# SohirMaskey/raincast-gnn

Hardware: AMD Instinct MI355X
Metric: training graphs/s (24h_mixed GNN, full train step) (higher is better)
Workload: dtype f32 (split-bf16x3 GEMM products, fp32 accumulate); 1 GPU; cfg2: 24h_mixed, 32 graphs x 500 stations, k=10, 4 GINE layers, D=128; global_batch=32, graphs_per_gpu=32, nodes_per_gpu=16000, edges_per_gpu=176000, parallelism=dp1, hip_graph=True, station_order=locality, allreduce_in_graph=False, allreduce_overlap=False, head_fold=True

## Files before the change

### raincast-gnn_amd/csrc/gine_chain.hip

```cpp
#include "gine_common.hpp"
#include "gine_slab.hpp"
#include "gine_wgrad.hpp"
#include "gine_chainfold.hpp"
#include "gine_chainrow.hpp"

#include <algorithm>

namespace gine {
namespace {

typedef float floatx16 __attribute__((ext_vector_type(16)));

constexpr int kRowTile = 32;

#ifdef GINE_CHAIN_PROFILE
__device__ long long g_chain_prof[1024][16];
#define CHAIN_MARK(i)                                                          \
  do {                                                                         \
    if (threadIdx.x == 0 && blockIdx.x < 1024)                                 \
      g_chain_prof[blockIdx.x][i] = (long long)__builtin_amdgcn_s_memtime();  \
  } while (0)
#define CHAIN_RT(i)                                                            \
  do {                                                                         \
    if (threadIdx.x == 0 && blockIdx.x < 1024)                                 \
// ... 74 lines not shown
    const int c = k < F ? k : (k < FP ? 0 : k - FP + F);
    const float v = WT[(size_t)c * D + col];
    bf[s] = (k >= F && k < FP) ? 0.f : v;
  }
}

struct TileRange {
  int first, end, step;
};
__device__ __forceinline__ TileRange tile_range(int num_tiles, int nb) {
  const int xcd = blockIdx.x % kNumXcd, pos = blockIdx.x / kNumXcd;
  const int here = nb / kNumXcd + (xcd < nb % kNumXcd ? 1 : 0);
  const int span = (num_tiles + kNumXcd - 1) / kNumXcd;
  const int b = xcd * span;
  return TileRange{b + pos, min(num_tiles, b + span), here};
}

template <int D, int FP, int KIND>
__global__ __launch_bounds__(2 * D) void k_chain(ChainArgs a, int64_t N, int num_tiles) {
  constexpr int NT = 2 * D;
  constexpr int D4 = D / 4;
  constexpr int LDA = D + 4;
  constexpr bool kDimRed = KIND == CH_F2;
  constexpr int K2 = kDimRed ? FP + D : D;
  constexpr int LDB = K2 + 4;
  constexpr int BOFF = kDimRed ? FP : 0;
  constexpr int ITEMS = kRowTile * D4 / NT;
  constexpr int RSTEP = NT / D4;
  constexpr int XITEMS = (kRowTile * FP + NT - 1) / NT;
  constexpr bool kF2D = KIND == CH_F2D, kB2D = KIND == CH_B2D;
  constexpr bool kMask = KIND == CH_B1 || kB2D;
  constexpr bool kX = kDimRed || kF2D;
  constexpr int LDC = FP + D + 4;
  __shared__ __attribute__((aligned(16))) float sA[kRowTile * LDA];
  __shared__ __attribute__((aligned(16))) float sB[kF2D ? 4 : kRowTile * LDB];
  __shared__ __attribute__((aligned(16))) float sC[kF2D ? kRowTile * LDC : 4];

  const int wave = threadIdx.x / kWave, lane = threadIdx.x % kWave;
  const int h = lane >> 5, c32 = lane & 31;
  const int col = wave * 32 + c32;
  const int q_me = threadIdx.x % D4, r_me = threadIdx.x / D4;
  CHAIN_RT(11);
  CHAIN_MARK(0);
  const int nb = gridDim.x;

  float bf1[D / 2], bf2[K2 / 2];
  const bool w16 =
      ((reinterpret_cast<uintptr_t>(a.w1) | reinterpret_cast<uintptr_t>(a.w2)) & 15) == 0;
  if constexpr (KIND == CH_F1) {
    if (w16) {
      frag_t4<D>(bf1, a.w1, D, col, h);
      frag_t4<D>(bf2, a.w2, D, col, h);
    } else {
      frag_t<D>(bf1, a.w1, D, col, h);
      frag_t<D>(bf2, a.w2, D, col, h);
    }
  } else if constexpr (kF2D) {
    if (w16) frag_t4<D>(bf1, a.w1, D, col, h);
    else frag_t<D>(bf1, a.w1, D, col, h);
  } else if constexpr (KIND == CH_F2) {
    frag_t<D>(bf1, a.w1, D, col, h);
  } else if constexpr (kMask) {
    frag_n<D>(bf1, a.w1, a.F + D, a.F, col, h);
  } else if constexpr (KIND == CH_B2) {
    frag_n<D>(bf1, a.w1, D, 0, col, h);
  }
// ... 51 lines not shown
    for (int i = 0; i < ITEMS; ++i) {
      const int r = r_me + i * RSTEP;
      const float4 v = (n0 + r < N) ? raw[i] : f4_zero();
      float* dst = &sA[r * LDA + 4 * q_me];
      *reinterpret_cast<float4*>(dst) = v;
    }
    if constexpr (kX) {
      float* sx = kF2D ? sC : sB;
      constexpr int LDX = kF2D ? LDC : LDB;
#pragma unroll
      for (int i = 0; i < XITEMS; ++i) {
        const int idx = threadIdx.x + i * NT;
        if (idx < kRowTile * FP) sx[(idx / FP) * LDX + idx % FP] = idx % FP < a.F ? xr[i] : 0.f;
      }
    }
    __syncthreads();
    if (kt < 2) CHAIN_MARK(2 + 4 * kt);
    if (tile + tr.step < tr.end) load_tile(tile + tr.step, raw, xr);

    floatx16 acc;
    acc = tile_mma<D>(sA, LDA, bf1, c32, h);
#pragma unroll
    for (int r = 0; r < 16; ++r) {
      const int rr = (r & 3) + 8 * (r >> 2) + 4 * h;
      const int64_t n = n0 + rr;
      float v = acc[r] + bias1;
      if constexpr (kB2D) v = ep[r] > 0.f ? acc[r] : 0.f;
      if constexpr (kF2D) {
        v = relu_nan(v);
        sC[rr * LDC + FP + col] = v;
      } else {
        sB[rr * LDB + BOFF + col] = v;
      }
      if (n < N) a.out1[n * D + col] = v;
    }
    if (kt < 2) CHAIN_MARK(3 + 4 * kt);
    __syncthreads();
    if (kt < 2) CHAIN_MARK(4 + 4 * kt);

    if constexpr (!kF2D) {
      acc = tile_mma<K2>(sB, LDB, bf2, c32, h);
#pragma unroll
      for (int r = 0; r < 16; ++r) {
        const int rr = (r & 3) + 8 * (r >> 2) + 4 * h;
        const int64_t n = n0 + rr;
        float v = acc[r] + bias2;
        if constexpr (KIND == CH_F1) v = relu_nan(v);
        if constexpr (KIND == CH_B1) v = ep[r] > 0.f ? v : 0.f;
        if (n < N) a.out2[n * D + col] = v;
      }
    } else {
      acc = tile_mma<FP + D>(sC, LDC, bf3, c32, h);
#pragma unroll
      for (int r = 0; r < 16; ++r) {
        const int64_t n = n0 + (r & 3) + 8 * (r >> 2) + 4 * h;
        if (n < N) a.out3[n * D + col] = acc[r] + bias3;
      }
    }
    if (kt < 2) CHAIN_MARK(5 + 4 * kt);
  }
  CHAIN_MARK(10);
  CHAIN_RT(12);
}

inline int chain_grid(int64_t N) {
  const int64_t tiles = ceil_div(N, kRowTile);
  return (int)std::max<int64_t>(1, std::min<int64_t>(tiles, kNumCu));
}

template <int D, int FP, int KIND>
int launch_chain(const ChainArgs& a, int64_t N, hipStream_t s) {
  const int tiles = (int)ceil_div(N, kRowTile);
  hipLaunchKernelGGL((k_chain<D, FP, KIND>), dim3(chain_grid(N)), dim3(2 * D), 0, s, a, N,
                     tiles);
  GINE_LAUNCH_STATUS();
  return GINE_OK;
}

template <int NZ>
struct ChainWgradSrc {
  static constexpr int kZ = NZ;
  const float* p[NZ];
  const float* q[NZ];
  const float* x;
  int D, F;
  struct Raw {
    float4 v;
  };
  struct Col {
    float keep[4];
  };
  template <int Z> __device__ int i_dim(int) const { return Z == 0 ? F + D : D; }
  template <int Z> __device__ Col p_col(int) const { return Col{{1.f, 1.f, 1.f, 1.f}}; }
  template <int Z> __device__ Col q_col(int q4) const {
    Col c{{1.f, 1.f, 1.f, 1.f}};
    if constexpr (Z == 0) {
#pragma unroll
      for (int j = 0; j < 4; ++j) c.keep[j] = 4 * q4 + j < F + D ? 1.f : 0.f;
    }
    return c;
  }
  template <int Z> __device__ Raw p_load(int64_t n, int q4) const {
    return Raw{reinterpret_cast<const float4*>(p[Z] + n * D)[q4]};
  }
  template <int Z> __device__ Raw q_load(int64_t n, int q4) const {
    if constexpr (Z == 0) {
      const int I = F + D;
      float v[4];
#pragma unroll
      for (int j = 0; j < 4; ++j) {
        const int c = min(4 * q4 + j, I - 1);
        const float* src = c < F ? x + n * F + c : q[0] + n * D + (c - F);
        v[j] = *src;
      }
// ... 395 lines not shown
```

### raincast-gnn_amd/csrc/gine_common.hpp

```cpp
#pragma once

#include <hip/hip_runtime.h>
#include <stdint.h>

#include "gine_hip.h"

#define GINE_RETURN_IF_HIP(expr)                                  \
  do {                                                            \
    hipError_t gine_e_ = (expr);                                  \
    if (gine_e_ != hipSuccess) return GINE_ERR_HIP_BASE + (int)gine_e_; \
  } while (0)


#define GINE_LAUNCH_STATUS() \
  do {                                                            \
    hipError_t gine_e_ = hipGetLastError();                       \
    if (gine_e_ != hipSuccess) return GINE_ERR_HIP_BASE + (int)gine_e_; \
  } while (0)

namespace gine {

constexpr int kWave = 64;
constexpr int kNumXcd = 8;
constexpr int kNumCu = 256;

inline hipStream_t as_stream(void* s) { return reinterpret_cast<hipStream_t>(s); }

__device__ __forceinline__ int xcd_remap(int bid, int nblocks) {
  const int q = nblocks / kNumXcd, r = nblocks % kNumXcd;
  const int xcd = bid % kNumXcd, pos = bid / kNumXcd;
  const int base = (xcd < r) ? xcd * (q + 1) : r * (q + 1) + (xcd - r) * q;
  return base + pos;
}

__device__ __forceinline__ float4 f4_zero() { return make_float4(0.f, 0.f, 0.f, 0.f); }

__device__ __forceinline__ float relu_nan(float v) { return __builtin_elementwise_maximum(v, 0.0f); }

__device__ __forceinline__ bool block_any(bool pred, int* word) {
  __syncthreads();
  if (threadIdx.x == 0) *word = 0;
  __syncthreads();
  if (pred) *word = 1;
  __syncthreads();
  const bool any = *word != 0;
  __syncthreads();
  return any;
}

template <bool FMA>
__device__ __forceinline__ float edge_lin(float a, float w, float b) {
  if constexpr (FMA) return __builtin_fmaf(a, w, b);
  return a * w + b;
}

__device__ __forceinline__ double shfl_xor_d(double v, int m) {
  return __shfl_xor(v, m, kWave);
}

__host__ __device__ inline int64_t ceil_div(int64_t a, int64_t b) { return (a + b - 1) / b; }

__device__ __forceinline__ void count_valid_parts(const float* __restrict__ y, int64_t n,
                                                  uint32_t* __restrict__ parts) {
  __shared__ uint32_t s_w[4];
  const int64_t chunk = (n + GINE_COUNT_PARTS - 1) / GINE_COUNT_PARTS;
  for (int p = blockIdx.x; p < GINE_COUNT_PARTS; p += gridDim.x) {
    const int64_t lo = (int64_t)p * chunk, hi = lo + chunk < n ? lo + chunk : n;
    uint32_t c = 0;
// ... 11 lines not shown
```

### raincast-gnn_amd/csrc/gine_deepset.hip

```cpp
#include "gine_common.hpp"
#include "gine_chainfold.hpp"
#include "gine_bf16x3.hpp"
#include "gine_chainrow.hpp"

#include <algorithm>
#include <type_traits>

namespace gine {
namespace {

typedef float floatx16 __attribute__((ext_vector_type(16)));

__host__ __device__ constexpr int tiles_per_group(int G, int M) { return (G * M + 15) / 16; }

#ifndef GINE_DS_BF16X3
#define GINE_DS_BF16X3 1
#endif
template <int KP>
struct DsImg {
  static constexpr int KX = (KP + 15) / 16 * 16;
  static constexpr int RS = KX + 8;
  static constexpr int PLANE = 32 * RS;
  static constexpr int FLOATS = 3 * PLANE / 2;
};
// ... 472 lines not shown
  float bf[H / 2];
  frag_n<H>(bf, a.w1, a.FX + H, a.FX, col, h);
  float ep[16];
#pragma unroll
  for (int r = 0; r < 16; ++r) {
    int64_t n = n0 + (r & 3) + 8 * (r >> 2) + 4 * h;
    n = n < N ? n : N - 1;
    ep[r] = a.u[n * H + col];
  }
#pragma unroll
  for (int i = 0; i < ITEMS; ++i) {
    const int r = r_me + i * RSTEP;
    *reinterpret_cast<float4*>(&sA[r * LDA + 4 * q_me]) = (n0 + r < N) ? raw[i] : f4_zero();
  }
  __syncthreads();
  floatx16 acc = tile_mma<H>(sA, LDA, bf, c32, h);
#pragma unroll
  for (int r = 0; r < 16; ++r) {
    const int rr = (r & 3) + 8 * (r >> 2) + 4 * h;
    const float v = ep[r] > 0.f ? acc[r] : 0.f;
    sB[rr * LDA + col] = v;
    if (n0 + rr < N) a.dt[(n0 + rr) * H + col] = v;
  }
  frag_n<H>(bf, a.w2, H, 0, col, h);
  __syncthreads();
  acc = tile_mma<H>(sB, LDA, bf, c32, h);
#pragma unroll
  for (int r = 0; r < 16; ++r) {
    const int rr = (r & 3) + 8 * (r >> 2) + 4 * h;
    s_dr[rr * H + col] = n0 + rr < N ? acc[r] + 0.f : 0.f;
  }
}

template <int H, int KP, int G, bool X3, bool CHAIN = false>
__device__ __forceinline__ bool ds_bwd_body(const float* __restrict__ ens,
                                            const uint16_t* __restrict__ mask,
                                            const float* __restrict__ dr,
                                            float* __restrict__ slab, int64_t N, int M, int F,
                                            int num_groups, float* s_lds,
                                            const DsChainArgs& ch = DsChainArgs{}) {
  static_assert(!CHAIN || G == 16, "a group is one chain tile at G = 16 only");
  constexpr int NT = 2 * H;
  constexpr int KI = ds_bwd_ki(KP);
  using I = DsBwdImg<KI>;
  constexpr int LD = X3 ? I::RS : KP + 4;
  constexpr int TILEF = X3 ? I::FLOATS : 32 * (KP + 4);
  constexpr int NIF = X3 ? KI / 32 : KP / 32;
  constexpr int TAIL = X3 ? 0 : KP - 32 * NIF;
  float* s_e0 = s_lds;
  float* s_e1 = s_lds + TILEF;
  float* s_dr = s_lds + 2 * TILEF;
  const int wave = threadIdx.x / kWave, lane = threadIdx.x % kWave;
  const int h = lane >> 5, c32 = lane & 31;
  const int col = wave * 32 + c32;
  if constexpr (X3) {
    uint16_t* i0 = reinterpret_cast<uint16_t*>(s_e0);
    uint16_t* i1 = reinterpret_cast<uint16_t*>(s_e1);
    const int w = (KI - F) * I::RS;
    for (int i = threadIdx.x; i < 3 * w; i += blockDim.x) {
      const int pl = i / w, e = F * I::RS + i % w;
      i0[pl * I::PLANE + e] = 0;
      i1[pl * I::PLANE + e] = 0;
    }
  } else {
    zero_pad<KP>(s_e0, F);
    zero_pad<KP>(s_e1, F);
// ... 76 lines not shown
        const float* erow = buf + (16 * h + q) * LD;
#pragma unroll
        for (int it = 0; it < NIF; ++it)
          gw[it] = __builtin_amdgcn_mfma_f32_32x32x2f32(dh[q], erow[32 * it + c32], gw[it], 0,
                                                        0, 0);
#pragma unroll
        for (int j = 0; j < TAIL; j += 4) {
          const float4 e4 = *reinterpret_cast<const float4*>(erow + 32 * NIF + j);
          tw[j] = __builtin_fmaf(dh[q], e4.x, tw[j]);
          tw[j + 1] = __builtin_fmaf(dh[q], e4.y, tw[j + 1]);
          tw[j + 2] = __builtin_fmaf(dh[q], e4.z, tw[j + 2]);
          tw[j + 3] = __builtin_fmaf(dh[q], e4.w, tw[j + 3]);
        }
      }
    }
    DS_MARK(3 + 0 * (int)gw[0][0]);
  };
  if constexpr (CHAIN) {
    float* sA = s_dr + 2 * G * H;
    walk_tiles<true, true>(gr, GM, tpg, st, ens, N * M, F, s_e0, s_e1, mask, tile, [&]() {
      ds_chain_tile<H>(ch, N, (int64_t)gr.first * 2 * G, sA, sA + 32 * (H + 4), s_dr, wave,
                       c32, h);
    });
  } else {
    walk_tiles<true, true>(gr, GM, tpg, st, ens, N * M, F, s_e0, s_e1, mask, tile);
  }
  if constexpr (X3) {
    bool bad = false;
#pragma unroll
    for (int it = 0; it < NIF; ++it) bad = bad || wave_any_nan(gw[it]);
    if (block_any(bad, reinterpret_cast<int*>(s_e0))) return false;
  }
  float* out = slab + (size_t)blockIdx.x * ((size_t)H * F + H);
#pragma unroll
  for (int it = 0; it < NIF; ++it) {
#pragma unroll
    for (int q = 0; q < 16; ++q) {
      const int o = wave * 32 + (q & 3) + 8 * (q >> 2) + 4 * h;
      if (32 * it + c32 < F) out[(size_t)o * F + 32 * it + c32] = gw[it][q];
    }
  }
#pragma unroll
  for (int j = 0; j < TAIL; ++j) {
    const float v = tw[j] + __shfl_xor(tw[j], 32, kWave);
    if (h == 0 && 32 * NIF + j < F) out[(size_t)col * F + 32 * NIF + j] = v;
  }
  gb += shfl_xor_d(gb, 32);
  if (h == 0) out[(size_t)H * F + col] = (float)gb;
  return true;
}

#ifndef GINE_DS_BWD_BF16X3
#define GINE_DS_BWD_BF16X3 0
#endif
template <int H, int KP, int G>
constexpr int ds_bwd_lds_floats() {
  constexpr int f32 = 2 * 32 * (KP + 4);
  constexpr int x3 = GINE_DS_BWD_BF16X3 ? 2 * DsBwdImg<ds_bwd_ki(KP)>::FLOATS : 0;
  return (f32 > x3 ? f32 : x3) + 2 * G * H;
}

template <int H, int KP, int G>
__global__ __launch_bounds__(2 * H) void k_deepset_bwd(const float* __restrict__ ens,
                                                       const uint16_t* __restrict__ mask,
                                                       const float* __restrict__ dr,
                                                       float* __restrict__ slab, int64_t N,
                                                       int M, int F, int num_groups) {
  __shared__ __attribute__((aligned(16))) float s_lds[ds_bwd_lds_floats<H, KP, G>()];
#if GINE_DS_BWD_BF16X3
  if (ds_bwd_body<H, KP, G, true>(ens, mask, dr, slab, N, M, F, num_groups, s_lds)) return;
  __syncthreads();
#endif
  ds_bwd_body<H, KP, G, false>(ens, mask, dr, slab, N, M, F, num_groups, s_lds);
}

template <int H, int KP>
__global__ __launch_bounds__(2 * H) void k_deepset_bwd_chain(const float* __restrict__ ens,
                                                             const uint16_t* __restrict__ mask,
                                                             DsChainArgs ch,
                                                             float* __restrict__ slab, int64_t N,
                                                             int M, int F, int num_groups) {
  __shared__ __attribute__((aligned(16)))
  float s_lds[ds_bwd_lds_floats<H, KP, 16>() + ds_chain_lds_floats<H>()];
#if GINE_DS_BWD_BF16X3
  if (ds_bwd_body<H, KP, 16, true, true>(ens, mask, nullptr, slab, N, M, F, num_groups, s_lds,
                                         ch))
    return;
  __syncthreads();
#endif
  ds_bwd_body<H, KP, 16, false, true>(ens, mask, nullptr, slab, N, M, F, num_groups, s_lds, ch);
}

// ... 322 lines not shown
```

### raincast-gnn_amd/csrc/gine_mpmlp.hip

```cpp
#include "gine_mpmlp.hpp"

namespace gine {
namespace {

template <bool FMA>
__global__ __launch_bounds__(kThreads, 1) void k_mp_fwd_mlp1(FusedArgs A) {
  __shared__ __attribute__((aligned(16))) FusedLds L;
  const TileSeq ts = tile_seq(A.num_tiles, blockIdx.x, gridDim.x);
  const int nt = ts.count();
  const int wave = __builtin_amdgcn_readfirstlane(threadIdx.x / kWave);
  if (wave < kMatThreads / kWave) matrix_role(A, L, ts, nt);
  else gather_role<FMA>(A, L, ts, nt);
}

#ifndef GINE_LW_U
#define GINE_LW_U 4
#endif
constexpr int kLwU = GINE_LW_U;
constexpr int kLwRowLoads = 9;
constexpr int kLwRowsMax = kLwRowLoads * (kThreads - kMatThreads) / kD4;
constexpr int kLwRegion = 73712;
struct LayerWinLds {
  float tt[4 * 32 * kTLD];
  double sr[2 * 8 * kD];
// ... 275 lines not shown
  for (int it = 0; it < kLayerTiles; ++it) {
    if (it >= nt) break;
    const int T = ts.at(it);
    const int lo = st.lo;
    st.store(L.win, tab, rpl, p, SP, kG, R);
    __syncthreads();
    LAYER_MARK_T(kMatThreads, 22 + it);
    if (it + 1 < nt) st.load(A, la, p, SP, kG);
    f4v self[kRowsPerHalf], acc[kRowsPerHalf];
    int c[kRowsPerHalf];
#pragma unroll
    for (int i = 0; i < kRowsPerHalf; ++i) {
      const int r = hw + kHalves * i;
      const int n = T * kTileRows + r;
      c[i] = rpl[r + 1] - rpl[r];
      self[i] = *reinterpret_cast<const f4v*>(wb + (min(n, N - 1) - lo) * (int)kRowBytes + qb);
      acc[i] = f4v_zero();
    }
    if (GINE_FUSED_DBG != 1)
      lw_sum<FMA>(acc, wb, tab + hw * SP, tab + (hw + kHalves) * SP, qb, SP, lw, lb, masked,
                  c[0], c[1]);
#pragma unroll
    for (int i = 0; i < kRowsPerHalf; ++i) {
      const int r = hw + kHalves * i;
      const int64_t n = (int64_t)T * kTileRows + r;
      const f4v zv = add_scaled(acc[i], ope, self[i]);
      uint32_t h0, m0, l0, h1, m1, l1;
      split2(zv.x, zv.y, h0, m0, l0);
      split2(zv.z, zv.w, h1, m1, l1);
      uint16_t* pl = L.planes[it & 1] + r * kPS + 4 * t;
      *reinterpret_cast<uint2*>(pl) = make_uint2(h0, h1);
      *reinterpret_cast<uint2*>(pl + kTileRows * kPS) = make_uint2(m0, m1);
      *reinterpret_cast<uint2*>(pl + 2 * kTileRows * kPS) = make_uint2(l0, l1);
      if (n < N) *reinterpret_cast<f4v*>(A.z + n * kD + 4 * t) = zv;
    }
    LAYER_MARK_T(kMatThreads, 14 + it);
    __syncthreads();
  }
  constexpr int kW2Per = kD * kD4 / kG;
  W2Regs<kW2Per> w2r;
  w2r.load(reinterpret_cast<const float4*>(B.W2), p, kG);
  __syncthreads();
  w2r.store(reinterpret_cast<float*>(L.win), p, kG);
  if (p < GINE_COUNT_PARTS)
    reinterpret_cast<uint32_t*>(reinterpret_cast<float*>(L.win) + kLwHeadOff + kHC)[p] = 0;
  __syncthreads();
}

template <bool FMA, int EPI, bool WIN = false>
__global__ __launch_bounds__(kThreads, 1) void k_mp_fwd_layer(FusedArgs A, LayerArgs B) {
  using Lds = std::conditional_t<WIN, LayerWinLds, LayerLds>;
  __shared__ __attribute__((aligned(16))) Lds L;
  const TileSeq ts = tile_seq(A.num_tiles, blockIdx.x, gridDim.x);
  const int nt = ts.count();
  const int tid = threadIdx.x;
  const int wave = __builtin_amdgcn_readfirstlane(tid / kWave);
  const bool mat = wave < kMatThreads / kWave;
  long long* phw = bnacc_phase(A.bnacc, 2 * kD);
  const long long ph = phw[0] + 1, consumed = phw[1 + ((ph - 1) & 1)];
  float* hwl;
  if constexpr (WIN) {
    hwl = reinterpret_cast<float*>(L.win) + kLwHeadOff;
  } else {
    hwl = L.hd;
  }
  uint32_t* const cwl = reinterpret_cast<uint32_t*>(hwl + kHC);
  if constexpr (!WIN)
    if (tid < GINE_COUNT_PARTS) cwl[tid] = 0;
// ... 545 lines not shown
```

### raincast-gnn_amd/csrc/gine_mpmlp.hpp

```cpp
#pragma once
#include "gine_common.hpp"
#include "gine_bnacc.hpp"
#include "gine_edge.hpp"
#include "gine_bf16x3.hpp"
#include "gine_headrow.hpp"
#include "gine_mlpsrc.hpp"

#include <algorithm>
#include <atomic>
#include <mutex>
#include <type_traits>

namespace gine {
namespace {

constexpr int kD = 128, kD4 = kD / 4;
constexpr int kTileRows = 32;
constexpr int kLD = kD + 4;
constexpr int kKS = kD / 2;
#ifndef GINE_FUSED_GATHER_WAVES
#define GINE_FUSED_GATHER_WAVES 8
#endif
constexpr int kMatThreads = 256;
constexpr int kGatherWaves = GINE_FUSED_GATHER_WAVES;
// ... 213 lines not shown
    if constexpr (LAYER) {
      if (it <= 2 && acc[0] == 1.2345e-30f) tt[0] = 0.f;
      if (it <= 2) LAYER_MARK(7 + 2 * it);
    }
#endif
#pragma unroll
    for (int r = 0; r < 16; ++r) tt[((r & 3) + 8 * (r >> 2) + 4 * h) * kTLD + c32] = acc[r];
    __builtin_amdgcn_wave_barrier();
    [[maybe_unused]] double st1[4], st2[4];
    if constexpr (!EVAL) {
#pragma unroll
      for (int k = 0; k < 4; ++k) {
        st1[k] = sr[(0 * 8 + grp) * kD + 32 * wave + 4 * cq + k];
        st2[k] = sr[(1 * 8 + grp) * kD + 32 * wave + 4 * cq + k];
      }
    }
#pragma unroll
    for (int i = 0; i < 4; ++i) {
      const int row = grp + 8 * i;
      const int64_t n = (int64_t)T * kTileRows + row;
      const float4 v = *reinterpret_cast<const float4*>(&tt[row * kTLD + 4 * cq]);
      if (n >= A.N) continue;
      const float vv[4] = {v.x, v.y, v.z, v.w};
      float o4[4];
#pragma unroll
      for (int k = 0; k < 4; ++k) {
        o4[k] = vv[k] + bb[k];
        if constexpr (!EVAL) {
          st1[k] += (double)o4[k];
          st2[k] += (double)o4[k] * (double)o4[k];
        }
      }
      if constexpr (!EVAL)
        *reinterpret_cast<float4*>(A.a1 + n * kD + 32 * wave + 4 * cq) =
            make_float4(o4[0], o4[1], o4[2], o4[3]);
      if constexpr (LAYER || EVAL)
        *reinterpret_cast<float4*>(&a1k[(it - 1) * kTileRows * kLD + row * kLD + 32 * wave +
                                        4 * cq]) = make_float4(o4[0], o4[1], o4[2], o4[3]);
    }
    if constexpr (!EVAL) {
#pragma unroll
      for (int k = 0; k < 4; ++k) {
        sr[(0 * 8 + grp) * kD + 32 * wave + 4 * cq + k] = st1[k];
        sr[(1 * 8 + grp) * kD + 32 * wave + 4 * cq + k] = st2[k];
      }
    }
    __builtin_amdgcn_wave_barrier();
    if constexpr (LAYER) {
      if (it <= 2) LAYER_MARK(8 + 2 * it);
    }
    __syncthreads();
  }
  if constexpr (EVAL) return;
  __builtin_amdgcn_wave_barrier();
  const int which = lane >> 5, cc = 32 * wave + (lane & 31);
  double s = 0.0;
#pragma unroll
  for (int g = 0; g < 8; ++g) s += sr[(which * 8 + g) * kD + cc];
  if (A.partials) A.partials[(size_t)blockIdx.x * 2 * kD + which * kD + cc] = s;
  if constexpr (LAYER) {
    bnacc_add<false>(A.bnacc, 2 * kD, which * kD + cc, s);
    asm volatile("s_waitcnt vmcnt(0)" ::: "memory");
    LAYER_MARK(13);
  } else if (A.bnacc) {
    bnacc_add(A.bnacc, 2 * kD, which * kD + cc, s);
  }
}

template <bool FMA, bool LAST_SYNC = true, bool PLANES = false, bool STORE_Z = true>
__device__ __forceinline__ void gather_role(const FusedArgs& A, FusedLds& L, const TileSeq& ts,
                                            int nt) {
  int p_;
  if constexpr (STORE_Z) p_ = threadIdx.x - kMatThreads;
  else p_ = per_round((int)threadIdx.x) - kMatThreads;
  const int p = p_;
  const int hw = p >> 5, t = p & 31;
  const int N = A.N;
  const uint32_t qb = (uint32_t)t * 16u;
  const char* xb = reinterpret_cast<const char*>(A.x);
  RowptrStage rp;
  EdgeStage es;
#pragma unroll
  for (int i = 0; i < kRowsPerHalf; ++i) {
    rp.beg[i] = rp.end[i] = 0;
    es.nbr[i] = 0;
    es.attr[i] = 0.f;
    es.cnt[i] = 0;
  }
  auto row_of = [&](int T, int i) { return T * kTileRows + hw + kHalves * i; };
  auto clamp_row = [&](int n) { return n < N ? n : N - 1; };
  auto issue_rowptr = [&](int T) {
#pragma unroll
    for (int i = 0; i < kRowsPerHalf; ++i) {
      const int n = clamp_row(row_of(T, i));
      rp.beg[i] = A.rowptr[n];
      rp.end[i] = A.rowptr[n + 1];
    }
  };
  auto issue_edges = [&](int T) {
#pragma unroll
    for (int i = 0; i < kRowsPerHalf; ++i) {
      const int cnt = row_of(T, i) < N ? min(rp.end[i] - rp.beg[i], kSlots) : 0;
      const int e = cnt > 0 ? rp.beg[i] + min(t, cnt - 1) : 0;
      es.nbr[i] = A.nbr[e];
// ... 38 lines not shown
        float a0[kU], a1v[kU];
#pragma unroll
        for (int u = 0; u < kU; ++u) {
          const int j = min(j0 + u, kSlots - 1);
          r0[u] = ld_f4v(xb, (uint32_t)L.nbr[hw][pr][j] * kRowBytes + qb);
          r1[u] = ld_f4v(xb, (uint32_t)L.nbr[hw][pr + 1][j] * kRowBytes + qb);
          a0[u] = L.attr[hw][pr][j];
          a1v[u] = L.attr[hw][pr + 1][j];
        }
#pragma unroll
        for (int u = 0; u < kU; ++u) {
          edge_acc<FMA>(acc[pr], r0[u], a0[u], lw, lb, j0 + u < cnt[pr]);
          edge_acc<FMA>(acc[pr + 1], r1[u], a1v[u], lw, lb, j0 + u < cnt[pr + 1]);
        }
      }
    }
#pragma unroll
    for (int i = 0; i < kRowsPerHalf; ++i) {
      const int r = hw + kHalves * i;
      const int64_t n = (int64_t)T * kTileRows + r;
      const f4v zv = add_scaled(acc[i], ope, self[i]);
      if constexpr (PLANES) {
        uint32_t h0, m0, l0, h1, m1, l1;
        split2(zv.x, zv.y, h0, m0, l0);
        split2(zv.z, zv.w, h1, m1, l1);
        uint16_t* pl = tile_planes(L, it) + r * kPS + 4 * t;
        *reinterpret_cast<uint2*>(pl) = make_uint2(h0, h1);
        *reinterpret_cast<uint2*>(pl + kTileRows * kPS) = make_uint2(m0, m1);
        *reinterpret_cast<uint2*>(pl + 2 * kTileRows * kPS) = make_uint2(l0, l1);
      } else {
        *reinterpret_cast<f4v*>(&sz[r * kLD + 4 * t]) = zv;
      }
      if constexpr (STORE_Z)
        if (n < N) *reinterpret_cast<f4v*>(A.z + n * kD + 4 * t) = zv;
    }
    if (it < 2) LAYER_MARK_T(kMatThreads, 14 + it);
    __builtin_amdgcn_wave_barrier();
    __syncthreads();
  }
  if constexpr (LAST_SYNC) __syncthreads();
}

constexpr int kLayerTiles = 2;
static_assert(kLayerTiles * 3 * kTileRows * kPS * 2 <= kD * kLD * 4, "planes fit in w");

template <int PER>
struct W2Regs {
  static_assert(PER == 8, "eight float4 per gather thread");
  float4 v0, v1, v2, v3, v4, v5, v6, v7;
  __device__ __forceinline__ void load(const float4* __restrict__ w4, int t, int n) {
    v0 = w4[t]; v1 = w4[t + n]; v2 = w4[t + 2 * n]; v3 = w4[t + 3 * n];
    v4 = w4[t + 4 * n]; v5 = w4[t + 5 * n]; v6 = w4[t + 6 * n]; v7 = w4[t + 7 * n];
  }
  __device__ __forceinline__ void put(float* w, int idx, float4 v) const {
    *reinterpret_cast<float4*>(&w[(idx / kD4) * kLD + 4 * (idx % kD4)]) = v;
  }
  __device__ __forceinline__ void store(float* w, int t, int n) const {
    put(w, t, v0); put(w, t + n, v1); put(w, t + 2 * n, v2); put(w, t + 3 * n, v3);
    put(w, t + 4 * n, v4); put(w, t + 5 * n, v5); put(w, t + 6 * n, v6); put(w, t + 7 * n, v7);
  }
};

struct LayerArgs {
  const float* W2;
  const float* b2;
  float* y;
  uint8_t* mask;
  BnFwdParams q;
// ... 35 lines not shown
```

### raincast-gnn_amd/csrc/gine_wgrad.hpp

```cpp
#pragma once

#include "gine_common.hpp"
#include "gine_bf16x3.hpp"

#ifndef GINE_WG_VARIANT
#define GINE_WG_VARIANT 0
#endif

namespace gine {

#if (GINE_WG_VARIANT & 8) != 0
__device__ unsigned long long gine_wg_clock[4096][4];
#endif

typedef float wg_floatx16 __attribute__((ext_vector_type(16)));

constexpr int kWgRows = 64;
constexpr int kWgTI = 128;
constexpr int kWgLdQ = kWgTI + 4;
#ifndef GINE_WG_TARGET_BLOCKS
#define GINE_WG_TARGET_BLOCKS 256
#endif
constexpr int kWgTargetBlocks = GINE_WG_TARGET_BLOCKS;
constexpr int kWgMinSubtiles = 2;
#ifndef GINE_WG_WAVES64
#define GINE_WG_WAVES64 8
#endif
constexpr int kWgWaves64 = GINE_WG_WAVES64;

#ifndef GINE_WG_BF16X3
#define GINE_WG_BF16X3 1
#endif

// ... 3 lines not shown
  static constexpr int kBytes = 3 * kPlane;
  __device__ static __forceinline__ int off(int c, int k) {
    return c * (kWgRows * 2) + 16 * ((k >> 3) ^ ((c >> 1) & 7)) + 2 * (k & 7);
  }
};

template <int TO>
constexpr size_t wg_lds_bytes() {
  constexpr size_t f32 = sizeof(float) * kWgRows * ((TO + 4) + kWgLdQ);
  constexpr size_t x3 = (size_t)3 * kWgRows * 2 * (TO + kWgTI);
  return GINE_WG_BF16X3 ? (f32 > x3 ? f32 : x3) : f32;
}

struct WgPlan {
  int tiles_o, tiles_i, chunks, rows_per_chunk;
};

inline WgPlan wg_plan(int64_t R, int O, int I, int Z, int TO, int total_tiles = 0) {
  WgPlan p;
  p.tiles_o = (int)ceil_div(O, TO);
  p.tiles_i = (int)ceil_div(I, kWgTI);
  const int64_t subtiles = ceil_div(R > 0 ? R : 1, kWgRows);
  if (total_tiles <= 0) total_tiles = Z * p.tiles_o * p.tiles_i;
  int64_t chunks = ceil_div(kWgTargetBlocks, (int64_t)total_tiles);
  const int64_t cap = ceil_div(subtiles, kWgMinSubtiles);
  if (chunks > cap) chunks = cap;
  if (chunks < 1) chunks = 1;
  const int64_t per = ceil_div(subtiles, chunks);
  p.rows_per_chunk = (int)(per * kWgRows);
  p.chunks = (int)ceil_div(R > 0 ? R : 1, p.rows_per_chunk);
  return p;
}

template <class Src, int Z, int TO, int NW>
__device__ __forceinline__ void wgrad_body(const Src& src, int64_t R, int O, int I, int chunk,
                                           int tile, int rows_per_chunk, size_t zstride,
                                           size_t cstride, float* __restrict__ slab,
                                           float* __restrict__ sP, float* __restrict__ sQ) {
  using Raw = typename Src::Raw;
  using Col = typename Src::Col;
#if (GINE_WG_VARIANT & 8) != 0
  const int blin = blockIdx.x + gridDim.x * blockIdx.y + gridDim.x * gridDim.y * blockIdx.z;
  if (threadIdx.x == 0 && blin < 4096) {
    gine_wg_clock[blin][0] = __builtin_amdgcn_s_memtime();
    gine_wg_clock[blin][1] = __builtin_amdgcn_s_memrealtime();
  }
#endif
  constexpr int NT = 64 * NW;
  constexpr int LDP = TO + 4;
  constexpr int PQ = TO / 4;
  constexpr int PG = NT / PQ;
  constexpr int PITEMS = kWgRows / PG;
  constexpr int QQ = kWgTI / 4, QG = NT / QQ;
  constexpr int QITEMS = kWgRows / QG;
  constexpr int NJ = NW == 8 ? 1 : 2;
  constexpr int NI = (NW == 4 && TO == 128) ? 2 : 1;
  static_assert(NW == 4 || (NW == 8 && TO == 64), "engine shapes");

  const int tiles_i = (int)ceil_div(I, kWgTI);
  const int o0 = (tile / tiles_i) * TO, i0 = (tile % tiles_i) * kWgTI;
  const int wave = __builtin_amdgcn_readfirstlane(threadIdx.x / kWave);
  const int lane = threadIdx.x % kWave;
  const int h = lane >> 5, c32 = lane & 31;
  const int ob = NW == 8 ? 32 * (wave >> 2) : (TO == 128 ? 64 * (wave >> 1) : 0);
  const int ib = NW == 8 ? 32 * (wave & 3) : (TO == 128 ? 64 * (wave & 1) : 32 * wave);
  const bool bias_block = (i0 == 0);
// ... 71 lines not shown
        if constexpr ((GINE_WG_VARIANT & 16) != 0) {
#pragma unroll
          for (int j = 0; j < NJ; ++j) an[j] = a[j] * 0.5f;
#pragma unroll
          for (int k = 0; k < NI; ++k) bn[k] = b[k] * 0.5f;
        } else {
#pragma unroll
          for (int j = 0; j < NJ; ++j) an[j] = pa[(s + 1) * LDP + 32 * j];
#pragma unroll
          for (int k = 0; k < NI; ++k) bn[k] = qb[(s + 1) * kWgLdQ + 32 * k];
        }
      }
      if (s % SP == 0 && s / SP < NITEMS) load_item(s / SP, n1);
      if constexpr ((GINE_WG_VARIANT & 1) == 0) {
#pragma unroll
        for (int j = 0; j < NJ; ++j)
#pragma unroll
          for (int k = 0; k < NI; ++k)
            acc[j][k] = __builtin_amdgcn_mfma_f32_32x32x2f32(a[j], b[k], acc[j][k], 0, 0, 0);
      }
      __builtin_amdgcn_sched_barrier(0);
#pragma unroll
      for (int j = 0; j < NJ; ++j) a[j] = an[j];
#pragma unroll
      for (int k = 0; k < NI; ++k) b[k] = bn[k];
    }
    __syncthreads();
  }

  float* out = slab + (size_t)Z * zstride + (size_t)chunk * cstride;
  if constexpr ((GINE_WG_VARIANT & 4) != 0) {
    if (acc[0][0][0] != 12345.f) return;
  }
#pragma unroll
  for (int k = 0; k < NI; ++k) {
    const int i = i0 + ib + 32 * k + c32;
    if (i >= I) continue;
#pragma unroll
    for (int j = 0; j < NJ; ++j) {
#pragma unroll
      for (int r = 0; r < 16; ++r) {
        const int o = o0 + ob + 32 * j + (r & 3) + 8 * (r >> 2) + 4 * h;
        if (o < O) out[(size_t)o * I + i] = acc[j][k][r];
      }
    }
  }
#if (GINE_WG_VARIANT & 8) != 0
  if (threadIdx.x == 0 && blin < 4096) {
    gine_wg_clock[blin][2] = __builtin_amdgcn_s_memtime();
    gine_wg_clock[blin][3] = __builtin_amdgcn_s_memrealtime();
  }
#endif
  if (bias_block) {
    double* sb = reinterpret_cast<double*>(sQ);
#pragma unroll
    for (int j = 0; j < 4; ++j) sb[pr * TO + 4 * pq + j] = bsum[j];
    __syncthreads();
    if ((int)threadIdx.x < TO && o0 + (int)threadIdx.x < O) {
      double t = 0.0;
#pragma unroll 8
      for (int g = 0; g < PG; ++g) t += sb[g * TO + threadIdx.x];
      out[(size_t)O * I + o0 + threadIdx.x] = (float)t;
    }
  }
}

template <int C, int ITEMS>
__device__ __forceinline__ void wg_store_cols(char* img, int cq, int k0, const float4 (&v)[ITEMS]) {
  static_assert(ITEMS == 2 || ITEMS == 4 || ITEMS == 8, "column runs");
  using Img = WgImg<C>;
#pragma unroll
  for (int e = 0; e < 4; ++e) {
    uint32_t ph[ITEMS / 2], pm[ITEMS / 2], pl[ITEMS / 2];
#pragma unroll
    for (int k = 0; k < ITEMS; k += 2) {
      const float a = e == 0 ? v[k].x : e == 1 ? v[k].y : e == 2 ? v[k].z : v[k].w;
      const float b = e == 0 ? v[k + 1].x : e == 1 ? v[k + 1].y : e == 2 ? v[k + 1].z : v[k + 1].w;
      split2(a, b, ph[k / 2], pm[k / 2], pl[k / 2]);
    }
    const int o = Img::off(4 * cq + e, k0);
    char* d[3] = {img + o, img + Img::kPlane + o, img + 2 * Img::kPlane + o};
    const uint32_t* src[3] = {ph, pm, pl};
#pragma unroll
    for (int pl3 = 0; pl3 < 3; ++pl3) {
      if constexpr (ITEMS == 2) {
        *reinterpret_cast<uint32_t*>(d[pl3]) = src[pl3][0];
      } else if constexpr (ITEMS == 4) {
        *reinterpret_cast<uint2*>(d[pl3]) = make_uint2(src[pl3][0], src[pl3][1]);
      } else {
        *reinterpret_cast<uint4*>(d[pl3]) =
            make_uint4(src[pl3][0], src[pl3][1], src[pl3][2], src[pl3][3]);
      }
    }
  }
}

// ... 107 lines not shown
      const int k0 = 16 * b + 8 * h;
      Bf16x3 fa[NJ], fb[NI];
#pragma unroll
      for (int j = 0; j < NJ; ++j) fa[j] = wg_col_frag<TO>(imgP, ob + 32 * j + c32, k0);
#pragma unroll
      for (int k = 0; k < NI; ++k) fb[k] = wg_col_frag<kWgTI>(imgQ, ib + 32 * k + c32, k0);
#pragma unroll
      for (int j = 0; j < NITEMS; ++j)
        if (j % KB == b) load_item(j, n1);
#pragma unroll
      for (int j = 0; j < NJ; ++j)
#pragma unroll
        for (int k = 0; k < NI; ++k) acc[j][k] = mfma_bf16x3(fa[j], fb[k], acc[j][k]);
      __builtin_amdgcn_sched_barrier(0);
    }
    __syncthreads();
  }

  bool bad = false;
#pragma unroll
  for (int j = 0; j < NJ; ++j)
#pragma unroll
    for (int k = 0; k < NI; ++k) bad = bad || wave_any_nan(acc[j][k]);
#ifndef GINE_WG_X3_NANCHECK
#define GINE_WG_X3_NANCHECK 1
#endif
  if (GINE_WG_X3_NANCHECK && block_any(bad, reinterpret_cast<int*>(imgP))) {
    wgrad_body<Src, Z, TO, NW>(src, R, O, I, chunk, tile, rows_per_chunk, zstride, cstride,
                               slab, sP, sQ);
    return;
  }

  float* out = slab + (size_t)Z * zstride + (size_t)chunk * cstride;
#pragma unroll
  for (int k = 0; k < NI; ++k) {
    const int i = i0 + ib + 32 * k + c32;
    if (i >= I) continue;
#pragma unroll
    for (int j = 0; j < NJ; ++j) {
#pragma unroll
      for (int r = 0; r < 16; ++r) {
        const int o = o0 + ob + 32 * j + (r & 3) + 8 * (r >> 2) + 4 * h;
        if (o < O) out[(size_t)o * I + i] = acc[j][k][r];
      }
    }
  }
  if (bias_block) {
    double* sb = reinterpret_cast<double*>(imgQ);
#pragma unroll
    for (int j = 0; j < 4; ++j) sb[pr * TO + 4 * pq + j] = bsum[j];
    __syncthreads();
    if ((int)threadIdx.x < TO && o0 + (int)threadIdx.x < O) {
      double t = 0.0;
#pragma unroll 8
      for (int g = 0; g < PG; ++g) t += sb[g * TO + threadIdx.x];
      out[(size_t)O * I + o0 + threadIdx.x] = (float)t;
    }
  }
}

template <bool X3, class Src, int Z, int TO, int NW>
__device__ __forceinline__ void wg_body(const Src& src, int64_t R, int O, int I, int chunk,
                                        int tile, int rows_per_chunk, size_t zstride,
                                        size_t cstride, float* __restrict__ slab, float* sP,
                                        float* sQ) {
  if constexpr (X3)
    wgrad_body_x3<Src, Z, TO, NW>(src, R, O, I, chunk, tile, rows_per_chunk, zstride, cstride,
                                  slab, sP, sQ);
  else
    wgrad_body<Src, Z, TO, NW>(src, R, O, I, chunk, tile, rows_per_chunk, zstride, cstride,
                               slab, sP, sQ);
}

template <class Src, int Z>
__device__ __forceinline__ int wg_tiles(const Src& src, int O, int I, int TO) {
  return (int)(ceil_div(O, TO) * ceil_div(src.template i_dim<Z>(I), kWgTI));
}

template <class Src, int TO, int NW, bool X3 = GINE_WG_BF16X3 != 0>
__device__ __forceinline__ void wgrad_block(const Src& src, int64_t R, int O, int I, int chunk,
                                            int y, int rows_per_chunk, size_t zstride,
                                            size_t cstride, float* __restrict__ slab,
                                            float* sP, float* sQ) {
  const int t0 = wg_tiles<Src, 0>(src, O, I, TO);
  if (y < t0) {
    wg_body<X3, Src, 0, TO, NW>(src, R, O, src.template i_dim<0>(I), chunk, y, rows_per_chunk,
                               zstride, cstride, slab, sP, sQ);
    return;
  }
  y -= t0;
// ... 53 lines not shown
```

Measured before the change: 71910 graphs/s.

## Use sc1 write-through 16-byte stores for activation, wgrad slab and deepset outputs

Result: no change. 72560 graphs/s (median of 6 runs) (+0.9%).

```diff
diff --git a/raincast-gnn_amd/csrc/gine_chain.hip b/raincast-gnn_amd/csrc/gine_chain.hip
--- a/raincast-gnn_amd/csrc/gine_chain.hip
+++ b/raincast-gnn_amd/csrc/gine_chain.hip
@@ -130,6 +130,9 @@
   constexpr bool kMask = KIND == CH_B1 || kB2D;
   constexpr bool kX = kDimRed || kF2D;
   constexpr int LDC = FP + D + 4;
+  static_assert(FP % 4 == 0 && LDC % 4 == 0, "u's columns of sC are 16-byte aligned");
+  constexpr bool kWtU16 = kF2D && wt_on(kWtD);
+  const bool wt_u = kWtU16 && (reinterpret_cast<uintptr_t>(a.out1) & 15) == 0;
   __shared__ __attribute__((aligned(16))) float sA[kRowTile * LDA];
   __shared__ __attribute__((aligned(16))) float sB[kF2D ? 4 : kRowTile * LDB];
   __shared__ __attribute__((aligned(16))) float sC[kF2D ? kRowTile * LDC : 4];
@@ -247,11 +250,22 @@
       } else {
         sB[rr * LDB + BOFF + col] = v;
       }
-      if (n < N) a.out1[n * D + col] = v;
+      if (!wt_u && n < N) a.out1[n * D + col] = v;
     }
     if (kt < 2) CHAIN_MARK(3 + 4 * kt);
     __syncthreads();
     if (kt < 2) CHAIN_MARK(4 + 4 * kt);
+    if constexpr (kWtU16) {
+      if (wt_u) {
+#pragma unroll
+        for (int i = 0; i < ITEMS; ++i) {
+          const int r = r_me + i * RSTEP;
+          if (n0 + r < N)
+            st_wt16(a.out1 + (n0 + r) * D + 4 * q_me,
+                    *reinterpret_cast<const float4*>(&sC[r * LDC + FP + 4 * q_me]));
+        }
+      }
+    }
 
     if constexpr (!kF2D) {
       acc = tile_mma<K2>(sB, LDB, bf2, c32, h);
@@ -295,6 +309,7 @@
 template <int NZ>
 struct ChainWgradSrc {
   static constexpr int kZ = NZ;
+  static constexpr int kWtGroup = kWtX;
   const float* p[NZ];
   const float* q[NZ];
   const float* x;
diff --git a/raincast-gnn_amd/csrc/gine_common.hpp b/raincast-gnn_amd/csrc/gine_common.hpp
--- a/raincast-gnn_amd/csrc/gine_common.hpp
+++ b/raincast-gnn_amd/csrc/gine_common.hpp
@@ -34,6 +34,71 @@
 }
 
 __device__ __forceinline__ float4 f4_zero() { return make_float4(0.f, 0.f, 0.f, 0.f); }
+
+#ifndef GINE_WT_STORES
+#define GINE_WT_STORES (1 | 2 | 4)
+#endif
+constexpr int kWtF = 1, kWtS = 2, kWtD = 4, kWtX = 8, kWtFZ = 16;
+constexpr bool wt_on(int group) { return (GINE_WT_STORES & group) != 0; }
+
+typedef float wt_f4 __attribute__((ext_vector_type(4)));
+__device__ __forceinline__ void st_wt16(float* p, wt_f4 v) {
+  asm volatile("global_store_dwordx4 %0, %1, off sc1\n\ts_nop 1" ::"v"(p), "v"(v) : "memory");
+}
+__device__ __forceinline__ void st_wt16(float* p, float4 v) {
+  st_wt16(p, wt_f4{v.x, v.y, v.z, v.w});
+}
+template <bool WT, class V>
+__device__ __forceinline__ void st16(float* p, V v) {
+  if constexpr (WT) st_wt16(p, v);
+  else *reinterpret_cast<V*>(p) = v;
+}
+__device__ __forceinline__ void wt_drain() { asm volatile("s_waitcnt vmcnt(0)" ::: "memory"); }
+
+constexpr int kWtLd = 36;
+template <class Acc>
+__device__ __forceinline__ void st_wt_block(float* tt, const Acc& acc, float* out, int64_t ld,
+                                            int o_first, int o_end, int i_first, int i_end,
+                                            int lane) {
+  const int h = lane >> 5, c32 = lane & 31;
+  const int cq = lane & 7, grp = lane >> 3;
+  const int64_t mis = (int64_t)((reinterpret_cast<uintptr_t>(out) >> 2) & 3);
+  float* outa = out - mis;
+  const int len = min(32, i_end - i_first);
+#pragma unroll
+  for (int r = 0; r < 16; ++r) {
+    const int row = (r & 3) + 8 * (r >> 2) + 4 * h;
+    const int sh = (int)((mis + (int64_t)(o_first + row) * ld + i_first) & 3);
+    tt[row * kWtLd + sh + c32] = acc[r];
+  }
+  __builtin_amdgcn_wave_barrier();
+  wt_f4 v[4];
+  float tail[4];
+#pragma unroll
+  for (int m = 0; m < 4; ++m) {
+    const int row = grp + 8 * m;
+    v[m] = *reinterpret_cast<const wt_f4*>(&tt[row * kWtLd + 4 * cq]);
+    tail[m] = tt[row * kWtLd + 32 + (cq & 3)];
+  }
+#pragma unroll
+  for (int m = 0; m < 4; ++m) {
+    const int row = grp + 8 * m;
+    if (o_first + row >= o_end) continue;
+    const int64_t s = mis + (int64_t)(o_first + row) * ld + i_first;
+    const int sh = (int)(s & 3);
+    float* g = outa + (s - sh);
+    const int lo = sh, hi = sh + len;
+    if (4 * cq >= lo && 4 * cq + 4 <= hi) {
+      st_wt16(g + 4 * cq, v[m]);
+    } else {
+#pragma unroll
+      for (int j = 0; j < 4; ++j)
+        if (4 * cq + j >= lo && 4 * cq + j < hi) g[4 * cq + j] = v[m][j];
+    }
+    if (cq < 4 && 32 + cq < hi) g[32 + cq] = tail[m];
+  }
+  __builtin_amdgcn_wave_barrier();
+}
 
 __device__ __forceinline__ float relu_nan(float v) { return __builtin_elementwise_maximum(v, 0.0f); }
 
diff --git a/raincast-gnn_amd/csrc/gine_deepset.hip b/raincast-gnn_amd/csrc/gine_deepset.hip
--- a/raincast-gnn_amd/csrc/gine_deepset.hip
+++ b/raincast-gnn_amd/csrc/gine_deepset.hip
@@ -528,6 +528,11 @@
   }
 }
 
+template <int H, int KP>
+constexpr int ds_bwd_wt_floats() {
+  return wt_on(kWtD) && H <= 128 && H * KP + H + 4 <= 8192 ? H * KP + H + 4 : 0;
+}
+
 template <int H, int KP, int G, bool X3, bool CHAIN = false>
 __device__ __forceinline__ bool ds_bwd_body(const float* __restrict__ ens,
                                             const uint16_t* __restrict__ mask,
@@ -670,6 +675,12 @@
     if (block_any(bad, reinterpret_cast<int*>(s_e0))) return false;
   }
   float* out = slab + (size_t)blockIdx.x * ((size_t)H * F + H);
+  constexpr bool kWt = ds_bwd_wt_floats<H, KP>() > 0;
+  const int mis = (int)((reinterpret_cast<uintptr_t>(out) >> 2) & 3);
+  if constexpr (kWt) {
+    __syncthreads();
+    out = s_lds + mis;
+  }
 #pragma unroll
   for (int it = 0; it < NIF; ++it) {
 #pragma unroll
@@ -685,6 +696,20 @@
   }
   gb += shfl_xor_d(gb, 32);
   if (h == 0) out[(size_t)H * F + col] = (float)gb;
+  if constexpr (kWt) {
+    __syncthreads();
+    float* outa = slab + (size_t)blockIdx.x * ((size_t)H * F + H) - mis;
+    const int end = mis + H * F + H;
+    for (int c = 4 * (int)threadIdx.x; c < end; c += 4 * NT) {
+      if (c >= mis && c + 4 <= end) {
+        st_wt16(outa + c, *reinterpret_cast<const wt_f4*>(&s_lds[c]));
+      } else {
+#pragma unroll
+        for (int j = 0; j < 4; ++j)
+          if (c + j >= mis && c + j < end) outa[c + j] = s_lds[c + j];
+      }
+    }
+  }
   return true;
 }
 
@@ -695,7 +720,8 @@
 constexpr int ds_bwd_lds_floats() {
   constexpr int f32 = 2 * 32 * (KP + 4);
   constexpr int x3 = GINE_DS_BWD_BF16X3 ? 2 * DsBwdImg<ds_bwd_ki(KP)>::FLOATS : 0;
-  return (f32 > x3 ? f32 : x3) + 2 * G * H;
+  constexpr int walk = (f32 > x3 ? f32 : x3) + 2 * G * H;
+  return walk > ds_bwd_wt_floats<H, KP>() ? walk : ds_bwd_wt_floats<H, KP>();
 }
 
 template <int H, int KP, int G>
diff --git a/raincast-gnn_amd/csrc/gine_mpmlp.hip b/raincast-gnn_amd/csrc/gine_mpmlp.hip
--- a/raincast-gnn_amd/csrc/gine_mpmlp.hip
+++ b/raincast-gnn_amd/csrc/gine_mpmlp.hip
@@ -331,8 +331,9 @@
       *reinterpret_cast<uint2*>(pl) = make_uint2(h0, h1);
       *reinterpret_cast<uint2*>(pl + kTileRows * kPS) = make_uint2(m0, m1);
       *reinterpret_cast<uint2*>(pl + 2 * kTileRows * kPS) = make_uint2(l0, l1);
-      if (n < N) *reinterpret_cast<f4v*>(A.z + n * kD + 4 * t) = zv;
-    }
+      if (n < N) st16<wt_on(kWtFZ)>(A.z + n * kD + 4 * t, zv);
+    }
+    if constexpr (wt_on(kWtFZ)) wt_drain();
     LAYER_MARK_T(kMatThreads, 14 + it);
     __syncthreads();
   }
diff --git a/raincast-gnn_amd/csrc/gine_mpmlp.hpp b/raincast-gnn_amd/csrc/gine_mpmlp.hpp
--- a/raincast-gnn_amd/csrc/gine_mpmlp.hpp
+++ b/raincast-gnn_amd/csrc/gine_mpmlp.hpp
@@ -269,8 +269,8 @@
         }
       }
       if constexpr (!EVAL)
-        *reinterpret_cast<float4*>(A.a1 + n * kD + 32 * wave + 4 * cq) =
-            make_float4(o4[0], o4[1], o4[2], o4[3]);
+        st16<wt_on(kWtF)>(A.a1 + n * kD + 32 * wave + 4 * cq,
+                          make_float4(o4[0], o4[1], o4[2], o4[3]));
       if constexpr (LAYER || EVAL)
         *reinterpret_cast<float4*>(&a1k[(it - 1) * kTileRows * kLD + row * kLD + 32 * wave +
                                         4 * cq]) = make_float4(o4[0], o4[1], o4[2], o4[3]);
@@ -307,6 +307,7 @@
 template <bool FMA, bool LAST_SYNC = true, bool PLANES = false, bool STORE_Z = true>
 __device__ __forceinline__ void gather_role(const FusedArgs& A, FusedLds& L, const TileSeq& ts,
                                             int nt) {
+  constexpr bool kWtZ = wt_on(PLANES ? kWtFZ : kWtF);
   int p_;
   if constexpr (STORE_Z) p_ = threadIdx.x - kMatThreads;
   else p_ = per_round((int)threadIdx.x) - kMatThreads;
@@ -411,8 +412,9 @@
         *reinterpret_cast<f4v*>(&sz[r * kLD + 4 * t]) = zv;
       }
       if constexpr (STORE_Z)
-        if (n < N) *reinterpret_cast<f4v*>(A.z + n * kD + 4 * t) = zv;
-    }
+        if (n < N) st16<kWtZ>(A.z + n * kD + 4 * t, zv);
+    }
+    if constexpr (STORE_Z && PLANES && kWtZ) wt_drain();
     if (it < 2) LAYER_MARK_T(kMatThreads, 14 + it);
     __builtin_amdgcn_wave_barrier();
     __syncthreads();
diff --git a/raincast-gnn_amd/csrc/gine_wgrad.hpp b/raincast-gnn_amd/csrc/gine_wgrad.hpp
--- a/raincast-gnn_amd/csrc/gine_wgrad.hpp
+++ b/raincast-gnn_amd/csrc/gine_wgrad.hpp
@@ -1,4 +1,6 @@
 #pragma once
+
+#include <type_traits>
 
 #include "gine_common.hpp"
 #include "gine_bf16x3.hpp"
@@ -68,6 +70,69 @@
   return p;
 }
 
+template <class Src, class = void>
+struct WgWtGroup {
+  static constexpr int value = kWtS;
+};
+template <class Src>
+struct WgWtGroup<Src, std::void_t<decltype(Src::kWtGroup)>> {
+  static constexpr int value = Src::kWtGroup;
+};
+template <class Src>
+constexpr bool wg_wt() { return wt_on(WgWtGroup<Src>::value); }
+
+template <bool WT, int NJ, int NI>
+__device__ __forceinline__ void wg_store_acc(const wg_floatx16 (&acc)[NJ][NI],
+                                             float* __restrict__ out, int O, int I, int ow,
+                                             int iw, float* lds, int wave, int lane) {
+  if constexpr (WT) {
+    float* tt = lds + wave * 32 * kWtLd;
+#pragma unroll
+    for (int k = 0; k < NI; ++k) {
+      if (iw + 32 * k >= I) continue;
+#pragma unroll
+      for (int j = 0; j < NJ; ++j) {
+        if (ow + 32 * j >= O) continue;
+        st_wt_block(tt, acc[j][k], out, (int64_t)I, ow + 32 * j, O, iw + 32 * k, I, lane);
+      }
+    }
+  } else {
+    const int h = lane >> 5, c32 = lane & 31;
+#pragma unroll
+    for (int k = 0; k < NI; ++k) {
+      const int i = iw + 32 * k + c32;
+      if (i >= I) continue;
+#pragma unroll
+      for (int j = 0; j < NJ; ++j) {
+#pragma unroll
+        for (int r = 0; r < 16; ++r) {
+          const int o = ow + 32 * j + (r & 3) + 8 * (r >> 2) + 4 * h;
+          if (o < O) out[(size_t)o * I + i] = acc[j][k][r];
+        }
+      }
+    }
+  }
+}
+
+template <int TO>
+__device__ __forceinline__ void wg_store_bias(float bt, float* brow, int o0, int O, float* lds) {
+  const int t = threadIdx.x;
+  const int sh = (int)(((reinterpret_cast<uintptr_t>(brow) >> 2) + o0) & 3);
+  if (t < TO) lds[sh + t] = bt;
+  __syncthreads();
+  const int hi = sh + min(TO, O - o0);
+  if (4 * t < hi && 4 * t + 4 > sh) {
+    float* g = brow + o0 - sh + 4 * t;
+    if (4 * t >= sh && 4 * t + 4 <= hi) {
+      st_wt16(g, *reinterpret_cast<const wt_f4*>(&lds[4 * t]));
+    } else {
+#pragma unroll
+      for (int j = 0; j < 4; ++j)
+        if (4 * t + j >= sh && 4 * t + j < hi) g[j] = lds[4 * t + j];
+    }
+  }
+}
+
 template <class Src, int Z, int TO, int NW>
 __device__ __forceinline__ void wgrad_body(const Src& src, int64_t R, int O, int I, int chunk,
                                            int tile, int rows_per_chunk, size_t zstride,
@@ -205,19 +270,7 @@
   if constexpr ((GINE_WG_VARIANT & 4) != 0) {
     if (acc[0][0][0] != 12345.f) return;
   }
-#pragma unroll
-  for (int k = 0; k < NI; ++k) {
-    const int i = i0 + ib + 32 * k + c32;
-    if (i >= I) continue;
-#pragma unroll
-    for (int j = 0; j < NJ; ++j) {
-#pragma unroll
-      for (int r = 0; r < 16; ++r) {
-        const int o = o0 + ob + 32 * j + (r & 3) + 8 * (r >> 2) + 4 * h;
-        if (o < O) out[(size_t)o * I + i] = acc[j][k][r];
-      }
-    }
-  }
+  wg_store_acc<wg_wt<Src>()>(acc, out, O, I, o0 + ob, i0 + ib, sP, wave, lane);
 #if (GINE_WG_VARIANT & 8) != 0
   if (threadIdx.x == 0 && blin < 4096) {
     gine_wg_clock[blin][2] = __builtin_amdgcn_s_memtime();
@@ -225,16 +278,20 @@
   }
 #endif
   if (bias_block) {
+    if constexpr (wg_wt<Src>()) __syncthreads();
     double* sb = reinterpret_cast<double*>(sQ);
 #pragma unroll
     for (int j = 0; j < 4; ++j) sb[pr * TO + 4 * pq + j] = bsum[j];
     __syncthreads();
+    float bt = 0.f;
     if ((int)threadIdx.x < TO && o0 + (int)threadIdx.x < O) {
       double t = 0.0;
 #pragma unroll 8
       for (int g = 0; g < PG; ++g) t += sb[g * TO + threadIdx.x];
-      out[(size_t)O * I + o0 + threadIdx.x] = (float)t;
-    }
+      bt = (float)t;
+      if constexpr (!wg_wt<Src>()) out[(size_t)O * I + o0 + threadIdx.x] = bt;
+    }
+    if constexpr (wg_wt<Src>()) wg_store_bias<TO>(bt, out + (size_t)O * I, o0, O, sP);
   }
 }
 
@@ -408,30 +465,22 @@
   }
 
   float* out = slab + (size_t)Z * zstride + (size_t)chunk * cstride;
-#pragma unroll
-  for (int k = 0; k < NI; ++k) {
-    const int i = i0 + ib + 32 * k + c32;
-    if (i >= I) continue;
-#pragma unroll
-    for (int j = 0; j < NJ; ++j) {
-#pragma unroll
-      for (int r = 0; r < 16; ++r) {
-        const int o = o0 + ob + 32 * j + (r & 3) + 8 * (r >> 2) + 4 * h;
-        if (o < O) out[(size_t)o * I + i] = acc[j][k][r];
-      }
-    }
-  }
+  wg_store_acc<wg_wt<Src>()>(acc, out, O, I, o0 + ob, i0 + ib, sP, wave, lane);
   if (bias_block) {
+    if constexpr (wg_wt<Src>()) __syncthreads();
     double* sb = reinterpret_cast<double*>(imgQ);
 #pragma unroll
     for (int j = 0; j < 4; ++j) sb[pr * TO + 4 * pq + j] = bsum[j];
     __syncthreads();
+    float bt = 0.f;
     if ((int)threadIdx.x < TO && o0 + (int)threadIdx.x < O) {
       double t = 0.0;
 #pragma unroll 8
       for (int g = 0; g < PG; ++g) t += sb[g * TO + threadIdx.x];
-      out[(size_t)O * I + o0 + threadIdx.x] = (float)t;
-    }
+      bt = (float)t;
+      if constexpr (!wg_wt<Src>()) out[(size_t)O * I + o0 + threadIdx.x] = bt;
+    }
+    if constexpr (wg_wt<Src>()) wg_store_bias<TO>(bt, out + (size_t)O * I, o0, O, sP);
   }
 }
 
```
